# proroklab/DVM-SLAM

Measured on AMD Instinct MI355X. Metric: frames/sec ORB extract+match 640x480x8lvl, higher is better.
Workload: dtype u8; 1 GPU; single agent tracking front end: 640x480 8-level ORB extract (1000 features) + frame-to-frame windowed Hamming match, one agent per GPU; frames_per_launch_group=256, resident_stream_frames=1024, nfeatures=1000, nlevels=8, ini_th_fast=20, min_th_fast=7, match=SearchByProjection(Cur,Last) window th=15, parallelism=agents1, pipeline_lanes=2, stream_texture=rich

## Files before the change

### dvm_slam_amd/csrc/capi.cpp

```cpp
#include <algorithm>
#include <cstring>
#include <new>
#include <string>
#include <type_traits>
#include <mutex>
#include <unordered_map>
#include <vector>

#include "../../include/dvmslam_hip.h"
#include "camera_model.h"
#include "chain.h"
#include "match_kernels.h"
#include "orb_pipeline.h"

namespace dvm {
const char* last_error_cstr();
}
using namespace dvm;

struct dvm_orb {
  OrbPipeline* p;
  float* d_scale = nullptr;
  uint64_t id = 0, serial = 0;
  int last_n = 0;
// ... 84 lines not shown
  if (rc == DVM_OK) h->last_n = nn;
  return rc;
}
int dvm_orb_last_result(dvm_orb* h, dvm_device_frame* out) {
  if (!h || !out) return DVM_ERR_INVALID;
  if (!h->p->configured || h->last_n < 0 || !h->id) { set_error("dvm_orb_last_result: no single-frame result on this handle"); return DVM_ERR_STATE; }
  OrbPipeline& P = *h->p;
  out->d_kps = reinterpret_cast<const dvm_keypoint*>(P.d_kps); out->d_desc = P.d_desc;
  out->n = h->last_n; out->device = P.device; out->handle_id = h->id; out->serial = h->serial;
  return DVM_OK;
}
int dvm_device_frame_valid(const dvm_device_frame* ref) {
  if (!ref || !ref->handle_id || !ref->d_kps) return 0;
  std::lock_guard<std::mutex> l(g_orb_live_mu);
  const auto it = g_orb_live.find(ref->handle_id);
  return it != g_orb_live.end() && it->second == ref->serial ? 1 : 0;
}
int dvm_orb_extract_batch_device(dvm_orb* h, const uint8_t* d_imgs, int batch, int rows, int cols, int stride,
                                 int64_t frame_stride, int lap0, int lap1) {
  if (!h) return DVM_ERR_INVALID;
  orb_result_changed(h, -1);
  return h->p->extract_device(d_imgs, batch, rows, cols, stride, frame_stride, lap0, lap1);
}
int dvm_orb_extract_batch_host(dvm_orb* h, const uint8_t* imgs, int batch, int rows, int cols, int stride,
                               int64_t frame_stride, int lap0, int lap1) {
  if (!h) return DVM_ERR_INVALID;
  orb_result_changed(h, -1);
  return h->p->extract_host(imgs, batch, rows, cols, stride, frame_stride, lap0, lap1);
}
int dvm_orb_staging(dvm_orb* h, int batch, int rows, int cols, uint8_t** host_ptr) {
  if (!h) return DVM_ERR_INVALID;
  return h->p->staging(batch, rows, cols, host_ptr);
}
int dvm_orb_extract_staged(dvm_orb* h, int batch, int rows, int cols, int lap0, int lap1) {
  if (!h) return DVM_ERR_INVALID;
  orb_result_changed(h, -1);
  return h->p->extract_staged(batch, rows, cols, lap0, lap1);
}
int dvm_orb_sync(dvm_orb* h) { return h ? h->p->sync() : DVM_ERR_INVALID; }
int dvm_orb_result_device(dvm_orb* h, int frame, const dvm_keypoint** d_kps, const uint8_t** d_desc,
                          const int32_t** d_n, int* capacity) {
  if (!h || !h->p->configured || frame < 0 || frame >= h->p->max_batch) return DVM_ERR_STATE;
  OrbPipeline& P = *h->p;
  if (d_kps) *d_kps = reinterpret_cast<const dvm_keypoint*>(P.d_kps + (size_t)frame * P.PD.kp_cap);
  if (d_desc) *d_desc = P.d_desc + (size_t)frame * P.PD.kp_cap * 32;
  if (d_n) *d_n = P.d_n + frame;
  if (capacity) *capacity = P.PD.kp_cap;
  return DVM_OK;
}
int dvm_orb_copy_result(dvm_orb* h, int frame, dvm_keypoint* d_kps_dst, uint8_t* d_desc_dst, int32_t* d_n_dst) {
  if (!h || !h->p->configured || frame < 0 || frame >= h->p->max_batch || !d_kps_dst || !d_desc_dst || !d_n_dst) return DVM_ERR_STATE;
  OrbPipeline& P = *h->p;
  const size_t cap = (size_t)P.PD.kp_cap;
  int rc = hip_check(hipMemcpyAsync(d_kps_dst, P.d_kps + (size_t)frame * cap, cap * sizeof(dvm_keypoint), hipMemcpyDeviceToDevice, P.stream), "copy kps");
  if (rc == DVM_OK) rc = hip_check(hipMemcpyAsync(d_desc_dst, P.d_desc + (size_t)frame * cap * 32, cap * 32, hipMemcpyDeviceToDevice, P.stream), "copy desc");
  if (rc == DVM_OK) rc = hip_check(hipMemcpyAsync(d_n_dst, P.d_n + frame, 4, hipMemcpyDeviceToDevice, P.stream), "copy n");
  return rc;
}
const float* dvm_orb_scale_factors_device(dvm_orb* h) { return h ? h->d_scale : nullptr; }
int dvm_orb_download(dvm_orb* h, int frame, dvm_keypoint* kps, uint8_t* desc, int cap, int* n, int* mono_index) {
  if (!h) return DVM_ERR_INVALID;
  return h->p->download(frame, kps, desc, cap, n, mono_index);
}
int dvm_orb_download_batch(dvm_orb* h, int count, dvm_keypoint* const* kps, uint8_t* const* desc, const int* caps, int* n, int* mono_index) {
  if (!h || !caps) return DVM_ERR_INVALID;
  return h->p->download_batch(count, kps, desc, caps, n, mono_index);
}
int dvm_orb_pyramid(dvm_orb* h, int frame, int level, const uint8_t** d_ptr, int* rows, int* cols, int* stride) {
  if (!h || !h->p->configured) return DVM_ERR_STATE;
  OrbPipeline& P = *h->p;
  if (level < 0 || level >= P.PD.nlevels || frame < 0 || frame >= P.max_batch) return DVM_ERR_INVALID;
  const LevelDesc& L = P.PD.lv[level];
  if (d_ptr) *d_ptr = P.d_pyr + (size_t)frame * P.PD.pyr_frame_bytes + L.pyr_off + (size_t)kEdge * L.stride + kEdge;
  if (rows) *rows = L.h;
  if (cols) *cols = L.w;
  if (stride) *stride = L.stride;
  return DVM_OK;
}

int dvm_orb_debug_level(dvm_orb* h, int frame, int level, int bordered, uint8_t* out) {
  if (!h || !h->p->configured || !out) return DVM_ERR_STATE;
  OrbPipeline& P = *h->p;
  if (level < 0 || level >= P.PD.nlevels || frame < 0 || frame >= P.last_batch) return DVM_ERR_INVALID;
  int rc = P.sync();
  if (rc != DVM_OK) return rc;
  const LevelDesc& L = P.PD.lv[level];
  const uint8_t* base = P.d_pyr + (size_t)frame * P.PD.pyr_frame_bytes + L.pyr_off;
  if (bordered)
    return hip_check(hipMemcpy2D(out, L.w + 2 * kEdge, base, L.stride, L.w + 2 * kEdge, L.h + 2 * kEdge, hipMemcpyDeviceToHost), "memcpy2d");
  return hip_check(hipMemcpy2D(out, L.w, base + (size_t)kEdge * L.stride + kEdge, L.stride, L.w, L.h, hipMemcpyDeviceToHost), "memcpy2d");
}
int dvm_orb_debug_blurred(dvm_orb* h, int frame, int level, uint8_t* out) {
  if (!h || !h->p->configured || !out) return DVM_ERR_STATE;
  OrbPipeline& P = *h->p;
  if (level < 0 || level >= P.PD.nlevels || frame < 0 || frame >= P.last_batch) return DVM_ERR_INVALID;
  int rc = P.refresh_blur();
  if (rc == DVM_OK) rc = P.sync();
  if (rc != DVM_OK) return rc;
  const LevelDesc& L = P.PD.lv[level];
  return hip_check(hipMemcpy2D(out, L.w, P.d_blur + (size_t)frame * P.PD.blur_frame_bytes + L.blur_off, L.blur_stride, L.w, L.h,
                               hipMemcpyDeviceToHost), "memcpy2d");
}
int dvm_orb_debug_candidates(dvm_orb* h, int frame, int level, int32_t* xs, int32_t* ys, int32_t* scores, int cap, int* n) {
  if (!h || !h->p->configured) return DVM_ERR_STATE;
  OrbPipeline& P = *h->p;
  if (level < 0 || level >= P.PD.nlevels || frame < 0 || frame >= P.last_batch) return DVM_ERR_INVALID;
  int rc = P.sync();
  if (rc != DVM_OK) return rc;
  const LevelDesc& LD = P.PD.lv[level];
  std::vector<int32_t> cc(std::max(LD.cell_count, 1));
// ... 57 lines not shown
  h->p->prof.enabled = enable != 0;
  h->p->prof.only_fast = enable == 2;
  return DVM_OK;
}
int dvm_orb_profile_get(dvm_orb* h, const char* name, double* total_ms, int64_t* launches) {
  if (!h || !name) return DVM_ERR_INVALID;
  if (total_ms) *total_ms = 0;
  if (launches) *launches = 0;
  return h->p->prof.get(name, total_ms, launches) ? DVM_OK : DVM_ERR_STATE;
}
int dvm_orb_profile_reset(dvm_orb* h) {
  if (!h) return DVM_ERR_INVALID;
  h->p->prof.reset();
  return DVM_OK;
}
void* dvm_orb_stream(dvm_orb* h) { return h ? (void*)h->p->stream : nullptr; }

int dvm_hamming_matrix(const uint8_t* A, int nA, const uint8_t* B, int nB, uint16_t* D, int on_device, void* stream) {
  if (nA < 0 || nB < 0 || (nA && !A) || (nB && !B)) return DVM_ERR_INVALID;
  if (nA == 0 || nB == 0) return DVM_OK;
  if (!D) return DVM_ERR_INVALID;
  int rc = need_device(0);
  if (on_device) {
    if (rc == DVM_ERR_NO_DEVICE) return rc;
    launch_hamming_matrix((hipStream_t)stream, A, nA, B, nB, D);
    return hip_check(hipGetLastError(), "hamming launch");
  }
  if (rc != DVM_OK) return rc;
  Stage st;
  const int iA = st.in(A, (size_t)nA * 32), iB = st.in(B, (size_t)nB * 32), oD = st.out(D, (size_t)nA * nB * 2);
  rc = st.upload();
  if (rc != DVM_OK) return rc;
  launch_hamming_matrix(nullptr, st.ptr<uint8_t>(iA), nA, st.ptr<uint8_t>(iB), nB, st.ptr<uint16_t>(oD));
  rc = hip_check(hipGetLastError(), "hamming launch");
  return rc == DVM_OK ? st.download() : rc;
}

int dvm_frame_create(int device, int capacity, int slots, dvm_frame** out) {
  if (!out || capacity < 1 || capacity > kFrameCap || slots < 1) {
    set_error("dvm_frame_create: capacity must be 1..8192, slots >= 1");
    return DVM_ERR_INVALID;
  }
  *out = nullptr;
  int rc = need_device(device);
  if (rc != DVM_OK) return rc;
  dvm_frame* f = new dvm_frame{};
  f->device = device; f->cap = capacity; f->slots = slots;
  FrameView& V = f->view;
  V.cap = capacity;
  const size_t S = (size_t)slots;
  rc = hip_check(hipMalloc(&V.skp, S * capacity * sizeof(float4)), "hipMalloc");
  if (rc == DVM_OK) rc = hip_check(hipMalloc(&V.sidx, S * capacity * 4), "hipMalloc");
  if (rc == DVM_OK) rc = hip_check(hipMalloc(&V.sdesc, S * capacity * 32), "hipMalloc");
  if (rc == DVM_OK) rc = hip_check(hipMalloc(&V.cellx_start, S * 80 * 4), "hipMalloc");
  if (rc == DVM_OK) rc = hip_check(hipMalloc(&V.n_sorted, S * 4), "hipMalloc");
  if (rc == DVM_OK) rc = hip_check(hipMalloc(&V.n_total, S * 4), "hipMalloc");
  if (rc == DVM_OK) rc = hip_check(hipMalloc(&V.n_overflow, 4), "hipMalloc");
  if (rc == DVM_OK) rc = hip_check(hipMemset(V.n_overflow, 0, 4), "memset");
  if (rc == DVM_OK) rc = hip_check(hipMemset(V.cellx_start, 0, S * 80 * 4), "memset");
  if (rc == DVM_OK) rc = hip_check(hipMemset(V.n_sorted, 0, S * 4), "memset");
  if (rc == DVM_OK) rc = hip_check(hipMemset(V.n_total, 0, S * 4), "memset");
  if (rc != DVM_OK) {
    dvm_frame_destroy(f);
    return rc;
  }
  *out = f;
  return DVM_OK;
}
void dvm_frame_destroy(dvm_frame* f) {
  if (!f) return;
  FrameView& V = f->view;
  if (V.skp) hipFree(V.skp);
  if (V.sidx) hipFree(V.sidx);
  if (V.sdesc) hipFree(V.sdesc);
  if (V.cellx_start) hipFree(V.cellx_start);
  if (V.n_sorted) hipFree(V.n_sorted);
  if (V.n_total) hipFree(V.n_total);
  if (V.n_overflow) hipFree(V.n_overflow);
  if (f->d_scratch) hipFree(f->d_scratch);
  delete f;
}
static int frame_bounds(dvm_frame* f, float minX, float maxX, float minY, float maxY) {
  if (!(maxX > minX) || !(maxY > minY)) {
    set_error("frame bounds empty");
    return DVM_ERR_INVALID;
  }
  FrameView& V = f->view;
  V.minX = minX; V.minY = minY;
  V.wInv = static_cast<float>(64) / static_cast<float>(maxX - minX);
  V.hInv = static_cast<float>(48) / static_cast<float>(maxY - minY);
  return DVM_OK;
}
int dvm_frame_build(dvm_frame* f, int slot, const dvm_keypoint* kps, const uint8_t* desc, int n, const int32_t* d_n,
                    float minX, float maxX, float minY, float maxY, int on_device, void* stream) {
  if (!f || slot < 0 || slot >= f->slots || n < 0 || n > f->cap || (n && (!kps || !desc))) return DVM_ERR_INVALID;
  int rc = frame_bounds(f, minX, maxX, minY, maxY);
  if (rc != DVM_OK) return rc;
  rc = hip_check(hipSetDevice(f->device), "hipSetDevice");
  if (rc != DVM_OK) return rc;
  if (on_device) {
    launch_frame_build((hipStream_t)stream, reinterpret_cast<const dvm_keypoint_pod*>(kps), 0, desc, 0, n, d_n, f->view, slot, 1);
    return hip_check(hipGetLastError(), "frame_build launch");
  }
  Stage st;
  const int iK = st.in_mapped(kps, (size_t)n * sizeof(dvm_keypoint)), iD = st.in_mapped(desc, (size_t)n * 32);
  rc = st.upload();
  if (rc != DVM_OK) return rc;
  launch_frame_build(st.stream(), st.ptr<dvm_keypoint_pod>(iK), 0, st.ptr<uint8_t>(iD), 0, n, nullptr, f->view, slot, 1);
  rc = hip_check(hipGetLastError(), "frame_build launch");
  return rc == DVM_OK ? hip_check(hipStreamSynchronize(st.stream()), "frame_build") : rc;
}
int dvm_frame_overflows(dvm_frame* f, int32_t* count) {
  if (!f || !count) return DVM_ERR_INVALID;
  int rc = hip_check(hipSetDevice(f->device), "hipSetDevice");
  if (rc != DVM_OK) return rc;
  rc = hip_check(hipMemcpy(count, f->view.n_overflow, 4, hipMemcpyDeviceToHost), "memcpy");
  if (rc != DVM_OK) return rc;
  if (*count) { set_error("frame grid: a device-side keypoint count exceeded the handle's capacity and was truncated"); return DVM_ERR_CAPACITY; }
  return DVM_OK;
}

int dvm_frame_build_batch(dvm_frame* f, int first_slot, int count, const dvm_keypoint* d_kps, int64_t kps_stride,
                          const uint8_t* d_desc, int64_t desc_stride, const int32_t* d_n, float minX, float maxX,
                          float minY, float maxY, void* stream) {
  if (!f || first_slot < 0 || count < 1 || first_slot + count > f->slots || !d_kps || !d_desc || !d_n) return DVM_ERR_INVALID;
  int rc = frame_bounds(f, minX, maxX, minY, maxY);
  if (rc != DVM_OK) return rc;
  launch_frame_build((hipStream_t)stream, reinterpret_cast<const dvm_keypoint_pod*>(d_kps), kps_stride, d_desc, desc_stride, 0,
// ... 814 lines not shown
```

### dvm_slam_amd/csrc/fuse_targets.cpp

```cpp
#include <cstring>
#include <new>
#include <string>

#include "../../include/dvmslam_hip.h"
#include "chain.h"
#include "fuse_targets_kernels.h"
#include "orb_pipeline.h"

using namespace dvm;

struct dvm_fuse_targets : Chain {
  size_t tgt_bytes = 0, grid_bytes = 0, pts_bytes = 0, res_bytes = 0;
  int max_points = 0, max_targets = 0, max_total = 0;
  int n_targets = -1;
  int build_timed = 0;
  float last_ms[2] = {0, 0};
};

namespace {
using Cursor64 = Cursor<64>;
constexpr int kMaxTargets = 65535;
constexpr int64_t kMaxEntries = (int64_t)1 << 27;
constexpr size_t kUpPerKeypoint = sizeof(dvm_keypoint_pod) + 32, kUpFixed = 2 * 64 * 4 + 4 * 64;
constexpr size_t kGridPerKeypoint = sizeof(float4) + 4 + 32, kGridFixed = 80 * 4 + 5 * 64;
constexpr size_t kPointBytes = 12 + 12 + 4 + 4 + 32 + 1;

int fail(const char* fn, int rc, const std::string& msg) { set_error(std::string(fn) + ": " + msg); return rc; }
}

extern "C" {

int dvm_fuse_targets_create(int device, dvm_fuse_targets** out) { return chain_create(device, out); }
void dvm_fuse_targets_destroy(dvm_fuse_targets* h) { chain_destroy(h); }

int dvm_fuse_targets_reserve(dvm_fuse_targets* h, int max_points, int max_targets, int max_total_target_keypoints) {
  if (!h || max_points < 0 || max_targets < 0 || max_targets > kMaxTargets || max_total_target_keypoints < 0 ||
      (int64_t)max_total_target_keypoints > (int64_t)max_targets * kFrameCap || (int64_t)max_points * max_targets > kMaxEntries)
    return fail("dvm_fuse_targets_reserve", DVM_ERR_INVALID, "bad sizes");
  if (max_points <= h->max_points && max_targets <= h->max_targets && max_total_target_keypoints <= h->max_total) return DVM_OK;
  DVM_HIP(hipSetDevice(h->device));
  DVM_HIP(hipStreamSynchronize(h->s));
  const int np = std::max(max_points, h->max_points), nt = std::max(max_targets, h->max_targets), tot = std::max(max_total_target_keypoints, h->max_total);
  if ((int64_t)np * nt > kMaxEntries) return fail("dvm_fuse_targets_reserve", DVM_ERR_INVALID, "bad sizes");
  h->tgt_bytes = h->grid_bytes = h->pts_bytes = h->res_bytes = 0; h->max_points = h->max_targets = h->max_total = 0; h->n_targets = -1;
  const size_t tgt = pad<64>(pad<64>((size_t)nt * sizeof(FtTargetDev)) + (size_t)tot * kUpPerKeypoint + (size_t)nt * kUpFixed);
  const size_t grid = pad<64>((size_t)tot * kGridPerKeypoint + (size_t)nt * kGridFixed + 64);
  const size_t pts = pad<64>((size_t)np * kPointBytes + 7 * 64 + pad<64>((size_t)np * nt));
  const size_t res = 2 * pad<64>((size_t)np * nt * 4);
  if (const char* what = h->ws.alloc(tgt + grid + pts + res, tgt + pts + res, tgt,  false,  false))
    return fail("dvm_fuse_targets_reserve", DVM_ERR_HIP, std::string(what) + " failed");
  h->tgt_bytes = tgt; h->grid_bytes = grid; h->pts_bytes = pts; h->res_bytes = res;
  h->max_points = np; h->max_targets = nt; h->max_total = tot;
  return DVM_OK;
}

int dvm_fuse_targets_profiling(dvm_fuse_targets* h, int enable) {
  if (!h) return DVM_ERR_INVALID;
  DVM_HIP(hipSetDevice(h->device));
  return h->timer.enable(enable != 0);
}
int dvm_fuse_targets_last_kernel_ms(dvm_fuse_targets* h, float* ms) {
  if (!h || !ms) return DVM_ERR_INVALID;
  ms[0] = h->last_ms[0]; ms[1] = h->last_ms[1];
  return DVM_OK;
}

int dvm_fuse_targets_set(dvm_fuse_targets* h, int n_targets, const dvm_ft_target* targets) {
  static_assert(sizeof(dvm_keypoint) == sizeof(dvm_keypoint_pod), "layout");
  const char* fn = "dvm_fuse_targets_set";
  if (!h || n_targets < 0 || (n_targets > 0 && !targets)) return fail(fn, DVM_ERR_INVALID, "missing argument");
  int64_t total = 0;
  for (int t = 0; t < n_targets; t++) {
    const dvm_ft_target& k = targets[t];
    const std::string w = "target " + std::to_string(t);
    if (k.n < 0 || k.n > kFrameCap) return fail(fn, DVM_ERR_INVALID, w + ": n outside [0, 8192]");
    if (k.n_levels < 1 || k.n_levels > 64) return fail(fn, DVM_ERR_INVALID, w + ": n_levels outside [1, 64]");
    if (!k.scale_factors || !k.inv_level_sigma2) return fail(fn, DVM_ERR_INVALID, w + ": missing level table");
    if (!(k.fx != 0.0f) || !(k.fy != 0.0f)) return fail(fn, DVM_ERR_INVALID, w + ": zero focal length");
    if (!(k.max_x > k.min_x) || !(k.max_y > k.min_y)) return fail(fn, DVM_ERR_INVALID, w + ": image bounds empty");
    if (k.n > 0 && (!k.kps || !k.desc)) return fail(fn, DVM_ERR_INVALID, w + ": missing keypoint array");
    for (int i = 0; i < k.n; i++)
      if ((uint32_t)k.kps[i].octave >= (uint32_t)k.n_levels) return fail(fn, DVM_ERR_INVALID, w + ": a keypoint's octave outside the level tables");
    total += k.n;
  }
  if (n_targets > h->max_targets || total > h->max_total)
    return fail(fn, DVM_ERR_CAPACITY, "beyond the reservation (dvm_fuse_targets_reserve): " + std::to_string(n_targets) + " targets with " +
                                          std::to_string(total) + " keypoints");
  h->n_targets = n_targets;
  if (n_targets == 0) return DVM_OK;
  DVM_HIP(hipSetDevice(h->device));
  DVM_HIP(hipStreamSynchronize(h->s));

  const WorkingSet& ws = h->ws;
  Cursor64 up{ws.hm, ws.d};
  Cursor64 grid{ws.d + h->tgt_bytes};
  FtTargetDev* tab = up.carve<FtTargetDev>((size_t)n_targets);
  int32_t* n_overflow = grid.carve<int32_t>(1);
  for (int t = 0; t < n_targets; t++) {
    const dvm_ft_target& k = targets[t];
    FtTargetDev& D = tab[t];
    std::memset(&D, 0, sizeof(D));
    const size_t n = (size_t)k.n;
    D.kps = reinterpret_cast<const dvm_keypoint_pod*>(up.put(k.kps, n * sizeof(dvm_keypoint_pod)));
    D.desc = up.put(k.desc, n * 32);
    D.sf = reinterpret_cast<const float*>(up.put(k.scale_factors, (size_t)k.n_levels * 4));
    D.inv_sigma2 = reinterpret_cast<const float*>(up.put(k.inv_level_sigma2, (size_t)k.n_levels * 4));
    D.n = k.n;
    FrameView& F = D.F;
    F.skp = grid.carve<float4>(n);
    F.sidx = grid.carve<int32_t>(n);
    F.sdesc = grid.carve<uint8_t>(n * 32);
    F.cellx_start = grid.carve<int32_t>(80);
    F.n_sorted = grid.carve<int32_t>(2);
    F.n_total = F.n_sorted + 1;
    F.n_overflow = n_overflow;
    F.cap = k.n;
    F.minX = k.min_x; F.minY = k.min_y;
    F.wInv = static_cast<float>(64) / static_cast<float>(k.max_x - k.min_x);
    F.hInv = static_cast<float>(48) / static_cast<float>(k.max_y - k.min_y);
    ProjectCam& C = D.C;
    std::memcpy(C.q, k.Tcw.q, 16); std::memcpy(C.t, k.Tcw.t, 12); std::memcpy(C.Ow, k.Ow, 12);
    C.fx = k.fx; C.fy = k.fy; C.cx = k.cx; C.cy = k.cy;
    C.min_x = k.min_x; C.max_x = k.max_x; C.min_y = k.min_y; C.max_y = k.max_y;
    C.log_scale_factor = k.log_scale_factor; C.n_levels = k.n_levels; C.sim3_pair = 0;
  }
  if (up.used() > h->tgt_bytes || grid.used() > h->grid_bytes) return fail(fn, DVM_ERR_STATE, "packed targets exceed the reserved regions");
  DVM_HIP(hipMemcpyAsync(ws.d, ws.hm, up.used(), hipMemcpyHostToDevice, h->s));
  DVM_HIP(h->timer.mark(0, h->s));
  launch_ft_build(h->s, reinterpret_cast<const FtTargetDev*>(ws.d), n_targets);
  DVM_HIP(h->timer.mark(1, h->s));
  h->build_timed = h->timer.on;
  return hip_check(hipGetLastError(), "dvm_fuse_targets_set launch");
}

int dvm_fuse_targets_run(dvm_fuse_targets* h, const dvm_ft_points* P, const uint8_t* skip, float th, int32_t* best_idx, int32_t* best_dist) {
  const char* fn = "dvm_fuse_targets_run";
  if (!h || !P) return fail(fn, DVM_ERR_INVALID, "missing argument");
  if (h->n_targets < 0) return fail(fn, DVM_ERR_INVALID, "no targets (dvm_fuse_targets_set comes first)");
  if (P->n < 0) return fail(fn, DVM_ERR_INVALID, "negative point count");
  if (P->n > h->max_points) return fail(fn, DVM_ERR_CAPACITY, "beyond the reservation (dvm_fuse_targets_reserve): " + std::to_string(P->n) + " points");
  const int T = h->n_targets, n = P->n;
  if (T == 0 || n == 0) return DVM_OK;
  if (!P->pos || !P->normal || !P->min_dist || !P->max_dist || !P->desc || !best_idx) return fail(fn, DVM_ERR_INVALID, "missing array");
  DVM_HIP(hipSetDevice(h->device));
  const size_t N = (size_t)n, E = N * (size_t)T;
  const WorkingSet& ws = h->ws;
  uint8_t* stage = ws.hm + h->tgt_bytes;
  uint8_t* dev = ws.d + h->tgt_bytes + h->grid_bytes;
  Cursor64 up{stage, dev};
  FtPoints A{};
  A.pos = reinterpret_cast<const float*>(up.put(P->pos, N * 12));
  A.normal = reinterpret_cast<const float*>(up.put(P->normal, N * 12));
  A.min_dist = reinterpret_cast<const float*>(up.put(P->min_dist, N * 4));
  A.max_dist = reinterpret_cast<const float*>(up.put(P->max_dist, N * 4));
  A.desc = up.put(P->desc, N * 32);
  A.valid = P->valid ? up.put(P->valid, N) : nullptr;
  A.skip = skip ? up.put(skip, E) : nullptr;
  A.n = n;
  if (up.used() > h->pts_bytes) return fail(fn, DVM_ERR_STATE, "packed points exceed the reserved region");
  int32_t* d_idx = reinterpret_cast<int32_t*>(dev + h->pts_bytes);
  int32_t* d_dist = reinterpret_cast<int32_t*>(dev + h->pts_bytes + pad<64>(E * 4));
  uint8_t* h_res = stage + h->pts_bytes;
  const size_t back = best_dist ? pad<64>(E * 4) + E * 4 : E * 4;

  DVM_HIP(hipMemcpyAsync(dev, stage, up.used(), hipMemcpyHostToDevice, h->s));
// ... 20 lines not shown
```

### dvm_slam_amd/csrc/match_device.h

```cpp
#pragma once
#include <hip/hip_runtime.h>
#include <stdint.h>

#include "match_kernels.h"

namespace dvm {

__device__ __forceinline__ void desc_load(const uint8_t* __restrict__ base, int idx, uint32_t (&w)[8]) {
  const uint4* q = reinterpret_cast<const uint4*>(base + (size_t)idx * 32);
  const uint4 a = q[0], b = q[1];
  w[0] = a.x; w[1] = a.y; w[2] = a.z; w[3] = a.w; w[4] = b.x; w[5] = b.y; w[6] = b.z; w[7] = b.w;
}
__device__ __forceinline__ int desc_distance(const uint32_t (&w)[8], const uint8_t* __restrict__ base, int idx) {
  const uint4* td = reinterpret_cast<const uint4*>(base + (size_t)idx * 32);
  const uint4 a = td[0], b = td[1];
  return __popc(a.x ^ w[0]) + __popc(a.y ^ w[1]) + __popc(a.z ^ w[2]) + __popc(a.w ^ w[3]) +
         __popc(b.x ^ w[4]) + __popc(b.y ^ w[5]) + __popc(b.z ^ w[6]) + __popc(b.w ^ w[7]);
}

template <class T>
__device__ __forceinline__ void top2_insert(T& k1, T& k2, T k) {
  k2 = min(k2, max(k1, k));
  k1 = min(k1, k);
}

template <int LANES, class Visit>
__device__ __forceinline__ void window_scan(const FrameView& F, float x, float y, float r, int minLevel, int maxLevel, int lane, Visit visit) {
  const int nMinCellX = max(0, (int)floorf((x - F.minX - r) * F.wInv));
  const int nMaxCellX = min(kGridCols - 1, (int)ceilf((x - F.minX + r) * F.wInv));
  const int nMinCellY = max(0, (int)floorf((y - F.minY - r) * F.hInv));
  const int nMaxCellY = min(kGridRows - 1, (int)ceilf((y - F.minY + r) * F.hInv));
  const bool empty = nMinCellX >= kGridCols || nMaxCellX < 0 || nMinCellY >= kGridRows || nMaxCellY < 0;
  if (empty || nMinCellX > nMaxCellX) return;
  const bool checkLevels = (minLevel > 0) || (maxLevel >= 0);
  const int beg = F.cellx_start[nMinCellX], end = F.cellx_start[nMaxCellX + 1];
  for (int p = beg + lane; p < end; p += LANES) {
    const float4 kp = F.skp[p];
    const int oct = __float_as_int(kp.z);
    const int iy = __float_as_int(kp.w) % kGridRows;
    if (iy < nMinCellY || iy > nMaxCellY) continue;
    if (checkLevels) {
      if (oct < minLevel) continue;
      if (maxLevel >= 0 && oct > maxLevel) continue;
    }
    const float dx = kp.x - x, dy = kp.y - y;
    if (!(fabsf(dx) < r && fabsf(dy) < r)) continue;
    visit(p, oct, dx, dy);
  }
}

#define DVM_ROW_DPP(v, CTRL, OLD) (uint32_t)__builtin_amdgcn_update_dpp(OLD, (int)(v), CTRL, 0xF, 0xF, false)
__device__ __forceinline__ uint32_t row_min(uint32_t k) {
  k = min(k, DVM_ROW_DPP(k, 0xB1, -1));
  k = min(k, DVM_ROW_DPP(k, 0x4E, -1));
  k = min(k, DVM_ROW_DPP(k, 0x141, -1));
  k = min(k, DVM_ROW_DPP(k, 0x140, -1));
  return k;
}
template <class T>
__device__ __forceinline__ void top2_merge(T& k1, T& k2, T o1, T o2) {
  const T n1 = min(k1, o1), n2 = min(max(k1, o1), min(k2, o2));
  k1 = n1; k2 = n2;
}
__device__ __forceinline__ void row_top2(uint32_t& k1, uint32_t& k2) {
  top2_merge(k1, k2, DVM_ROW_DPP(k1, 0xB1, 0), DVM_ROW_DPP(k2, 0xB1, 0));
  top2_merge(k1, k2, DVM_ROW_DPP(k1, 0x4E, 0), DVM_ROW_DPP(k2, 0x4E, 0));
  top2_merge(k1, k2, DVM_ROW_DPP(k1, 0x141, 0), DVM_ROW_DPP(k2, 0x141, 0));
  top2_merge(k1, k2, DVM_ROW_DPP(k1, 0x140, 0), DVM_ROW_DPP(k2, 0x140, 0));
}
#undef DVM_ROW_DPP
__device__ __forceinline__ uint32_t wave_min(uint32_t k) {
#pragma unroll
  for (int o = 32; o >= 1; o >>= 1) k = min(k, (uint32_t)__shfl_xor((int)k, o));
  return k;
}
template <class T>
__device__ __forceinline__ void wave_top2(T& k1, T& k2) {
#pragma unroll
  for (int o = 32; o >= 1; o >>= 1) {
    const T o1 = __shfl_xor(k1, o), o2 = __shfl_xor(k2, o);
    top2_merge(k1, k2, o1, o2);
  }
}
__device__ __forceinline__ int wave_sum(int v) {
#pragma unroll
  for (int o = 32; o >= 1; o >>= 1) v += __shfl_xor(v, o);
  return v;
}
__device__ __forceinline__ void block_sum4_put(int v, int* s4) {
  v = wave_sum(v);
  if ((threadIdx.x & 63) == 0) s4[threadIdx.x >> 6] = v;
}
__device__ __forceinline__ int block_sum4(const int* s4) { return s4[0] + s4[1] + s4[2] + s4[3]; }

template <class ORDER>
__device__ __forceinline__ int fv_find(const int32_t* __restrict__ fv_node, int fv_n, int32_t node) {
  int lo = 0, hi = fv_n;
  while (lo < hi) {
    const int mid = (lo + hi) >> 1;
    if ((ORDER)fv_node[mid] < (ORDER)node) lo = mid + 1; else hi = mid;
// ... 33 lines not shown
```

### dvm_slam_amd/csrc/match_kernels.h

```cpp
#pragma once
#include <hip/hip_runtime.h>
#include <stdint.h>

#include "orb_kernels.h"
#include "tri_model.h"
#include "undistort_f64.h"

struct dvm_frame;

namespace dvm {

constexpr int kFrameCap = 8192;

struct dvm_match_pod {
  int32_t best_idx, best_dist, second_dist;
  int16_t best_level, second_level;
};

constexpr int kGridCols = 64, kGridRows = 48;

struct FrameView {
  float4* skp;
  int32_t* sidx;
  uint8_t* sdesc;
  int32_t* cellx_start;
  int32_t* n_sorted;
  int32_t* n_total;
  int32_t* n_overflow;
  int32_t cap;
  float minX, minY, wInv, hInv;
  __host__ __device__ FrameView slot(int s) const {
    FrameView v = *this;
    v.skp += (int64_t)s * cap;
    v.sidx += (int64_t)s * cap;
    v.sdesc += (int64_t)s * cap * 32;
    v.cellx_start += (int64_t)s * 80;
    v.n_sorted += s;
    v.n_total += s;
    return v;
  }
};

struct PairQueries {
  const dvm_keypoint_pod* kps;
  const uint8_t* desc;
  const int32_t* n;
  int64_t kps_stride, desc_stride;
  const dvm_keypoint_pod* carry_kps;
  const uint8_t* carry_desc;
  const int32_t* carry_n;
  int32_t* n_out;
  int32_t cap;
};

struct FrustumFrame {
  float Rcw[9], tcw[3], Ow[3], fx, fy, cx, cy, min_x, max_x, min_y, max_y, bf, log_scale_factor;
  int32_t n_levels;
};
struct TrackPoint {
  float proj_x, proj_y, proj_xr, depth, view_cos;
  int32_t level, in_view;
};
struct TriPair {
  double cos_parallax_max;
  float K1[4], K2[4], T1w[12], T2w[12], Ow1[3], Ow2[3];
  float ratio_factor, th_far;
  int32_t far_points, n_levels;
};
struct ProjectCam {
  float q[4], t[3];
  float Ow[3], fx, fy, cx, cy, min_x, max_x, min_y, max_y, log_scale_factor;
  int32_t n_levels;
  int32_t sim3_pair;
  float q2[4], t2[3];
  float th;
};
struct Projection {
  float u, v, radius;
  int32_t level;
};
struct CamParams {
  float p[8];
};
struct TriGeom {
  float F12[9], ep[2];
  int32_t coarse, th_low;
};
struct TriGeomKB8 {
  float ep[2];
// ... 57 lines not shown
```

### dvm_slam_amd/csrc/orb_kernels.h

```cpp
#pragma once
#include <hip/hip_runtime.h>
#include <stdint.h>

#include "orb_device.h"

namespace dvm {

struct dvm_keypoint_pod {
  float x, y, size, angle, response;
  int32_t octave, class_id;
};

struct HostMirror {
  dvm_keypoint_pod* kps = nullptr;
  uint8_t* desc = nullptr;
  int32_t* n = nullptr;
  int32_t* mono = nullptr;
};

void upload_constants(const int8_t* disc_u, const int8_t* disc_v, const int* gauss7);
void launch_pyr_level0(hipStream_t s, const uint8_t* d_src, int rows, int cols, int sstride, int64_t frame_stride,
                       uint8_t* d_pyr, const PipelineDesc& PD, int batch);
void launch_pyr_resize(hipStream_t s, uint8_t* d_pyr, const PipelineDesc& PD, int level, const int32_t* d_tabs, int batch);
void launch_pyr_borders(hipStream_t s, uint8_t* d_pyr, const PipelineDesc& PD, int batch);
void launch_fast(hipStream_t s, const uint8_t* d_pyr, const CellDesc* d_cells, const PipelineDesc& PD, uint32_t* d_cand,
                 int32_t* d_cell_count, int batch, int max_rw, int max_rh, int cell_first, int cell_num, const CellDesc* h_cells);
int octree_root_nodes(const LevelDesc& L);
bool raise_dynamic_lds(const void* fn, int bytes);
bool octree_fits_device(const PipelineDesc& PD);
bool octree_prepare_device(const PipelineDesc& PD);
void launch_octree(hipStream_t s, const uint32_t* d_cand, const int32_t* d_cell_count, const CellDesc* d_cells, uint32_t* d_dense,
                   int32_t* d_lvl_count, const PipelineDesc& PD, int32_t* d_nid, uint32_t* d_sel, int32_t* d_nsel, int32_t* d_err,
                   int batch, int level_first, int level_num, bool latency = false);
bool octree_blur_fits(const PipelineDesc& PD);
void launch_octree_blur(hipStream_t s, const uint32_t* d_cand, const int32_t* d_cell_count, const CellDesc* d_cells, uint32_t* d_dense,
                        int32_t* d_lvl_count, const PipelineDesc& PD, int32_t* d_nid, uint32_t* d_sel, int32_t* d_nsel, int32_t* d_err, int batch,
                        const uint8_t* d_pyr, uint8_t* d_blur, const TileDesc* d_tiles, const int* gauss7);
void launch_assemble(hipStream_t s, const uint32_t* d_sel, const int32_t* d_nsel, const PipelineDesc& PD, int lap0,
                     int lap1, dvm_keypoint_pod* d_kps, KpAux* d_aux, int32_t* d_n, int32_t* d_mono, int batch,
                     HostMirror hm = HostMirror());
void launch_blur(hipStream_t s, const uint8_t* d_pyr, uint8_t* d_blur, const TileDesc* d_tiles, const PipelineDesc& PD,
                 const int32_t* d_lvl_start, int batch);
void launch_orient_desc(hipStream_t s, const uint8_t* d_pyr, const uint8_t* d_blur, const PipelineDesc& PD,
                        const KpAux* d_aux, const int32_t* d_n, dvm_keypoint_pod* d_kps, uint8_t* d_desc, int batch,
                        HostMirror hm = HostMirror());
void launch_orient_desc_blur(hipStream_t s, const uint8_t* d_pyr, const PipelineDesc& PD, const KpAux* d_aux, const int32_t* d_n,
                             dvm_keypoint_pod* d_kps, uint8_t* d_desc, int batch, HostMirror hm = HostMirror());

}
```

### dvm_slam_amd/csrc/orb_kernels.hip

```cpp
#include <hip/hip_runtime.h>

#include <map>
#include <mutex>
#include <utility>

#include <algorithm>
#include <cstdlib>

#include "orb_device.h"
#include "orb_kernels.h"
#include "blur_tile.h"

#pragma clang fp contract(off)

namespace dvm {

__constant__ int c_pattern[1024] = {
#include "orb_pattern_31.inc"
};
__constant__ int8_t c_circle[16][2] = {{0, 3},  {1, 3},   {2, 2},   {3, 1},   {3, 0},  {3, -1}, {2, -2}, {1, -3},
                                       {0, -3}, {-1, -3}, {-2, -2}, {-3, -1}, {-3, 0}, {-3, 1}, {-2, 2}, {-1, 3}};
__device__ uint2 c_disc_w[256];
__device__ uint2 c_disc_w43[512];
__constant__ int c_gauss7[7];
// ... 1321 lines not shown
  if (!h_cells || lds1_max <= 0) { launch_fast_wide(s, d_pyr, d_cells, PD, d_cand, d_cell_count, batch, max_rw, max_rh, cell_first, cell_num); return; }
  const int end = cell_first + cell_num;
  int run_first = cell_first, run_kind = -1, run_rw = 0, run_rh = 0;
  auto flush = [&](int upto) {
    if (upto <= run_first || run_kind < 0) return;
    const int n = upto - run_first;
    if (run_kind == 0) { launch_fast_wide(s, d_pyr, d_cells, PD, d_cand, d_cell_count, batch, run_rw, run_rh, run_first, n); return; }
    const int pitch = run_kind;
    const int lds = fast1_lds_layout(pitch, run_rw, run_rh).total();
    const dim3 grid(n * 8 * ((batch + 8 * kFastFramesPerWG - 1) / (8 * kFastFramesPerWG)));
    if (pitch == 48)
      hipLaunchKernelGGL((k_fast_cells1<48>), grid, dim3(64), lds, s, d_pyr, PD.pyr_frame_bytes, d_cells, PD, d_cand, d_cell_count, run_rw, run_rh, batch, run_first, n);
    else
      hipLaunchKernelGGL((k_fast_cells1<64>), grid, dim3(64), lds, s, d_pyr, PD.pyr_frame_bytes, d_cells, PD, d_cand, d_cell_count, run_rw, run_rh, batch, run_first, n);
  };
  int c = cell_first;
  while (c < end) {
    const int lvl = h_cells[c].level;
    int e = c, rw = 8, rh = 8;
    for (; e < end && h_cells[e].level == lvl; e++) { rw = std::max<int>(rw, h_cells[e].rw); rh = std::max<int>(rh, h_cells[e].rh); }
    const int pitch = fast1_pick_pitch(rw);
    const int kind = pitch != 0 && fast1_lds_layout(pitch, rw, rh).total() <= (pitch == 48 ? lds1_max : lds1_max64) ? pitch : 0;
    if (kind != 0 && kind == run_kind) {
      const int jrw = std::max(run_rw, rw), jrh = std::max(run_rh, rh);
      if (fast1_lds_layout(kind, jrw, jrh).total() > (kind == 48 ? lds1_max : lds1_max64)) { flush(c); run_first = c; run_kind = -1; }
    }
    if (kind != run_kind) { flush(c); run_first = c; run_kind = kind; run_rw = rw; run_rh = rh; }
    else { run_rw = std::max(run_rw, rw); run_rh = std::max(run_rh, rh); }
    c = e;
  }
  flush(end);
}
void launch_assemble(hipStream_t s, const uint32_t* d_sel, const int32_t* d_nsel, const PipelineDesc& PD, int lap0,
                     int lap1, dvm_keypoint_pod* d_kps, KpAux* d_aux, int32_t* d_n, int32_t* d_mono, int batch, HostMirror hm) {
  hipLaunchKernelGGL(k_assemble, dim3(batch), dim3(256), 0, s, d_sel, d_nsel, PD, lap0, lap1, d_kps, d_aux, d_n, d_mono, hm);
}
void launch_blur(hipStream_t s, const uint8_t* d_pyr, uint8_t* d_blur, const TileDesc* d_tiles, const PipelineDesc& PD,
                 const int32_t* d_lvl_start, int batch) {
  hipLaunchKernelGGL(k_blur7, dim3(xcd_grid(PD.ntiles, batch)), dim3(256), 0, s, d_pyr, PD.pyr_frame_bytes, d_blur,
                     PD.blur_frame_bytes, d_tiles, PD, d_lvl_start, batch);
}
void launch_orient_desc(hipStream_t s, const uint8_t* d_pyr, const uint8_t* d_blur, const PipelineDesc& PD,
                        const KpAux* d_aux, const int32_t* d_n, dvm_keypoint_pod* d_kps, uint8_t* d_desc, int batch, HostMirror hm) {
  hipLaunchKernelGGL(k_orient_desc, dim3(xcd_grid(cdiv(PD.kp_cap, 4 * kDescPerWave), batch)), dim3(256), 0, s, d_pyr, PD.pyr_frame_bytes,
                     d_blur, PD.blur_frame_bytes, PD, d_aux, d_n, d_kps, d_desc, batch, hm);
}

void launch_orient_desc_blur(hipStream_t s, const uint8_t* d_pyr, const PipelineDesc& PD, const KpAux* d_aux, const int32_t* d_n,
                             dvm_keypoint_pod* d_kps, uint8_t* d_desc, int batch, HostMirror hm) {
  hipLaunchKernelGGL(k_orient_desc_blur, dim3(xcd_grid(cdiv(PD.kp_cap, 4 * kPbPerWave), batch)), dim3(256), 0, s, d_pyr, PD.pyr_frame_bytes, PD,
                     d_aux, d_n, d_kps, d_desc, batch, hm);
}

}
```

### dvm_slam_amd/csrc/proj_device.h

```cpp
#pragma once
#include <hip/hip_runtime.h>
#include <stdint.h>

#include "camera_model.h"
#include "match_device.h"
#include "match_kernels.h"
#include "pose_f32.h"

namespace dvm {

constexpr uint32_t kInvalidKey = 0xFFFFFFFFu;

__device__ __forceinline__ void frame_build_block(const dvm_keypoint_pod* __restrict__ kps, const uint8_t* __restrict__ desc, int n,
                                                  const FrameView& F) {
  __shared__ uint32_t keys[kFrameCap];
  const int tid = threadIdx.x;
  int P = 64;
  while (P < n) P <<= 1;
  for (int i = tid; i < P; i += 1024) {
    uint32_t key = kInvalidKey;
    if (i < n) {
      const dvm_keypoint_pod kp = kps[i];
      int px = (int)roundf((kp.x - F.minX) * F.wInv);
      int py = (int)roundf((kp.y - F.minY) * F.hInv);
      if (px >= 0 && px < kGridCols && py >= 0 && py < kGridRows) key = ((uint32_t)(px * kGridRows + py) << 13) | (uint32_t)i;
    }
    keys[i] = key;
  }
  __syncthreads();
  for (int k = 2; k <= P; k <<= 1) {
    for (int j = k >> 1; j > 0; j >>= 1) {
      for (int i = tid; i < P; i += 1024) {
        int ixj = i ^ j;
        if (ixj > i) {
          uint32_t a = keys[i], b = keys[ixj];
          bool up = ((i & k) == 0);
          if ((a > b) == up) { keys[i] = b; keys[ixj] = a; }
        }
      }
      const int jn = j > 1 ? (j >> 1) : k;
      if (j >= 64 || jn >= 64) {
        __syncthreads();
      } else {
        __builtin_amdgcn_fence(__ATOMIC_ACQ_REL, "wavefront");
        __builtin_amdgcn_wave_barrier();
      }
    }
  }
  __shared__ int s_m;
  if (tid == 0) {
    int lo = 0, hi = P;
    while (lo < hi) {
      int mid = (lo + hi) >> 1;
      if (keys[mid] == kInvalidKey) hi = mid; else lo = mid + 1;
    }
    s_m = lo;
    *F.n_sorted = lo;
    *F.n_total = n;
  }
  __syncthreads();
  const int m = s_m;
  if (tid <= kGridCols) {
    uint32_t want = (uint32_t)(tid * kGridRows) << 13;
    int lo = 0, hi = m;
    while (lo < hi) {
      int mid = (lo + hi) >> 1;
      if (keys[mid] < want) lo = mid + 1; else hi = mid;
    }
    F.cellx_start[tid] = lo;
  }
  for (int p = tid; p < m; p += 1024) {
    const uint32_t key = keys[p];
    const int i = (int)(key & 0x1FFFu);
    const dvm_keypoint_pod kp = kps[i];
    F.skp[p] = make_float4(kp.x, kp.y, __int_as_float(kp.octave), __int_as_float((int)(key >> 13)));
    F.sidx[p] = i;
    const uint4* s = reinterpret_cast<const uint4*>(desc + (size_t)i * 32);
    uint4* d = reinterpret_cast<uint4*>(F.sdesc + (size_t)p * 32);
    d[0] = s[0];
    d[1] = s[1];
  }
}

__device__ __forceinline__ void window_top2(const FrameView& F, float x, float y, float r, int minLevel, int maxLevel,
                                            const uint8_t* __restrict__ qdesc32, const uint8_t* __restrict__ skip,
                                            const float* __restrict__ gate_inv_sigma2, double gate, int lane, uint32_t& k1_out,
                                            uint32_t& k2_out) {
  uint32_t k1 = (256u << 16) | 0xFFFFu, k2 = k1;
  uint32_t w[8];
  desc_load(qdesc32, 0, w);
  window_scan<16>(F, x, y, r, minLevel, maxLevel, lane, [&](int p, int oct, float dx, float dy) {
    if (skip && skip[F.sidx[p]]) return;
    if (gate_inv_sigma2) {
      const float e2 = __fadd_rn(__fmul_rn(dx, dx), __fmul_rn(dy, dy));
      if ((double)__fmul_rn(e2, gate_inv_sigma2[oct]) > gate) return;
    }
    top2_insert(k1, k2, ((uint32_t)desc_distance(w, F.sdesc, p) << 16) | (uint32_t)p);
  });
  row_top2(k1, k2);
  k1_out = k1; k2_out = k2;
}

struct ProjectRow {
  uint32_t k1, k2;
  float u, v, r;
  int level;
};
template <int MODEL = dvm_cam::kPinhole>
__device__ __forceinline__ ProjectRow project_row(const FrameView& F, const uint8_t* __restrict__ skip, const ProjectCam& C, float th,
                                                  const float* __restrict__ P, const float* __restrict__ normal,
                                                  const float* __restrict__ min_dist, const float* __restrict__ max_dist,
                                                  const uint8_t* __restrict__ desc, bool ok, int i, const float* __restrict__ scale_factors,
                                                  const float* __restrict__ gate_inv_sigma2, double gate, int lane,
                                                  const float* kb8 = nullptr) {
  float out_u = -1.f, out_v = -1.f, out_r = 0.f;
  int out_level = -1;
  const float p0 = P[3 * i], p1 = P[3 * i + 1], p2 = P[3 * i + 2];
  const float pw[3] = {p0, p1, p2};
  float pc[3];
  dvm_pose::se3_apply(C.q, C.t, pw, pc);
  float X = pc[0], Y = pc[1], Z = pc[2];
  float u, v;
// ... 48 lines not shown
```

Measured before the change: 291,100 frames/s.

## Index match grid per cell and compact window candidates via DPP prefix queue

Replaces the per-column start index with a full per-cell start table built with a branchless binary search, so window scans visit only keypoints in the covered rows of each column. A wave-level DPP prefix sum compacts candidate indices into a shared-memory queue so lanes work on dense candidate lists rather than filtering whole columns. Also replaces the three device-to-device memcpys in result copying with a single vectorized copy kernel. It adds shared memory use, wave barriers and a larger cell table in exchange for fewer wasted keypoint loads.

```diff
diff --git a/dvm_slam_amd/csrc/capi.cpp b/dvm_slam_amd/csrc/capi.cpp
--- a/dvm_slam_amd/csrc/capi.cpp
+++ b/dvm_slam_amd/csrc/capi.cpp
@@ -160,10 +160,11 @@
   if (!h || !h->p->configured || frame < 0 || frame >= h->p->max_batch || !d_kps_dst || !d_desc_dst || !d_n_dst) return DVM_ERR_STATE;
   OrbPipeline& P = *h->p;
   const size_t cap = (size_t)P.PD.kp_cap;
-  int rc = hip_check(hipMemcpyAsync(d_kps_dst, P.d_kps + (size_t)frame * cap, cap * sizeof(dvm_keypoint), hipMemcpyDeviceToDevice, P.stream), "copy kps");
-  if (rc == DVM_OK) rc = hip_check(hipMemcpyAsync(d_desc_dst, P.d_desc + (size_t)frame * cap * 32, cap * 32, hipMemcpyDeviceToDevice, P.stream), "copy desc");
-  if (rc == DVM_OK) rc = hip_check(hipMemcpyAsync(d_n_dst, P.d_n + frame, 4, hipMemcpyDeviceToDevice, P.stream), "copy n");
-  return rc;
+  int rc = hip_check(hipSetDevice(P.device), "hipSetDevice");
+  if (rc != DVM_OK) return rc;
+  launch_copy_result(P.stream, P.d_kps + (size_t)frame * cap, reinterpret_cast<dvm_keypoint_pod*>(d_kps_dst), P.d_desc + (size_t)frame * cap * 32, d_desc_dst,
+                     (int)cap, P.d_n + frame, d_n_dst);
+  return hip_check(hipGetLastError(), "copy_result launch");
 }
 const float* dvm_orb_scale_factors_device(dvm_orb* h) { return h ? h->d_scale : nullptr; }
 int dvm_orb_download(dvm_orb* h, int frame, dvm_keypoint* kps, uint8_t* desc, int cap, int* n, int* mono_index) {
@@ -327,12 +328,12 @@
   rc = hip_check(hipMalloc(&V.skp, S * capacity * sizeof(float4)), "hipMalloc");
   if (rc == DVM_OK) rc = hip_check(hipMalloc(&V.sidx, S * capacity * 4), "hipMalloc");
   if (rc == DVM_OK) rc = hip_check(hipMalloc(&V.sdesc, S * capacity * 32), "hipMalloc");
-  if (rc == DVM_OK) rc = hip_check(hipMalloc(&V.cellx_start, S * 80 * 4), "hipMalloc");
+  if (rc == DVM_OK) rc = hip_check(hipMalloc(&V.cell_start, S * kCellStartStride * 4), "hipMalloc");
   if (rc == DVM_OK) rc = hip_check(hipMalloc(&V.n_sorted, S * 4), "hipMalloc");
   if (rc == DVM_OK) rc = hip_check(hipMalloc(&V.n_total, S * 4), "hipMalloc");
   if (rc == DVM_OK) rc = hip_check(hipMalloc(&V.n_overflow, 4), "hipMalloc");
   if (rc == DVM_OK) rc = hip_check(hipMemset(V.n_overflow, 0, 4), "memset");
-  if (rc == DVM_OK) rc = hip_check(hipMemset(V.cellx_start, 0, S * 80 * 4), "memset");
+  if (rc == DVM_OK) rc = hip_check(hipMemset(V.cell_start, 0, S * kCellStartStride * 4), "memset");
   if (rc == DVM_OK) rc = hip_check(hipMemset(V.n_sorted, 0, S * 4), "memset");
   if (rc == DVM_OK) rc = hip_check(hipMemset(V.n_total, 0, S * 4), "memset");
   if (rc != DVM_OK) {
@@ -348,7 +349,7 @@
   if (V.skp) hipFree(V.skp);
   if (V.sidx) hipFree(V.sidx);
   if (V.sdesc) hipFree(V.sdesc);
-  if (V.cellx_start) hipFree(V.cellx_start);
+  if (V.cell_start) hipFree(V.cell_start);
   if (V.n_sorted) hipFree(V.n_sorted);
   if (V.n_total) hipFree(V.n_total);
   if (V.n_overflow) hipFree(V.n_overflow);
diff --git a/dvm_slam_amd/csrc/fuse_targets.cpp b/dvm_slam_amd/csrc/fuse_targets.cpp
--- a/dvm_slam_amd/csrc/fuse_targets.cpp
+++ b/dvm_slam_amd/csrc/fuse_targets.cpp
@@ -22,7 +22,7 @@
 constexpr int kMaxTargets = 65535;
 constexpr int64_t kMaxEntries = (int64_t)1 << 27;
 constexpr size_t kUpPerKeypoint = sizeof(dvm_keypoint_pod) + 32, kUpFixed = 2 * 64 * 4 + 4 * 64;
-constexpr size_t kGridPerKeypoint = sizeof(float4) + 4 + 32, kGridFixed = 80 * 4 + 5 * 64;
+constexpr size_t kGridPerKeypoint = sizeof(float4) + 4 + 32, kGridFixed = (size_t)kCellStartStride * 4 + 5 * 64;
 constexpr size_t kPointBytes = 12 + 12 + 4 + 4 + 32 + 1;
 
 int fail(const char* fn, int rc, const std::string& msg) { set_error(std::string(fn) + ": " + msg); return rc; }
@@ -110,7 +110,7 @@
     F.skp = grid.carve<float4>(n);
     F.sidx = grid.carve<int32_t>(n);
     F.sdesc = grid.carve<uint8_t>(n * 32);
-    F.cellx_start = grid.carve<int32_t>(80);
+    F.cell_start = grid.carve<int32_t>(kCellStartStride);
     F.n_sorted = grid.carve<int32_t>(2);
     F.n_total = F.n_sorted + 1;
     F.n_overflow = n_overflow;
diff --git a/dvm_slam_amd/csrc/match_device.h b/dvm_slam_amd/csrc/match_device.h
--- a/dvm_slam_amd/csrc/match_device.h
+++ b/dvm_slam_amd/csrc/match_device.h
@@ -24,6 +24,28 @@
   k1 = min(k1, k);
 }
 
+#define DVM_ROW_SHR(v, N) __builtin_amdgcn_update_dpp(0, v, 0x110 + N, 0xF, 0xF, false)
+template <int LANES>
+__device__ __forceinline__ int lanes_prefix(int v, int lane) {
+  static_assert(LANES == 16 || LANES == 64, "a DPP row or the wave");
+  v += DVM_ROW_SHR(v, 1);
+  v += DVM_ROW_SHR(v, 2);
+  v += DVM_ROW_SHR(v, 4);
+  v += DVM_ROW_SHR(v, 8);
+  if constexpr (LANES == 64) {
+    const int t0 = __builtin_amdgcn_readlane(v, 15), t1 = __builtin_amdgcn_readlane(v, 31), t2 = __builtin_amdgcn_readlane(v, 47);
+    v += (lane >= 16 ? t0 : 0) + (lane >= 32 ? t1 : 0) + (lane >= 48 ? t2 : 0);
+  }
+  return v;
+}
+#undef DVM_ROW_SHR
+template <int LANES>
+__device__ __forceinline__ int lanes_total(int incl) {
+  if constexpr (LANES == 64) return __builtin_amdgcn_readlane(incl, 63);
+  else return __builtin_amdgcn_update_dpp(0, incl, 0x15F, 0xF, 0xF, false);
+}
+
+constexpr int kWindowQueue = 4;
 template <int LANES, class Visit>
 __device__ __forceinline__ void window_scan(const FrameView& F, float x, float y, float r, int minLevel, int maxLevel, int lane, Visit visit) {
   const int nMinCellX = max(0, (int)floorf((x - F.minX - r) * F.wInv));
@@ -31,21 +53,42 @@
   const int nMinCellY = max(0, (int)floorf((y - F.minY - r) * F.hInv));
   const int nMaxCellY = min(kGridRows - 1, (int)ceilf((y - F.minY + r) * F.hInv));
   const bool empty = nMinCellX >= kGridCols || nMaxCellX < 0 || nMinCellY >= kGridRows || nMaxCellY < 0;
-  if (empty || nMinCellX > nMaxCellX) return;
+  if (empty || nMinCellX > nMaxCellX || nMinCellY > nMaxCellY) return;
   const bool checkLevels = (minLevel > 0) || (maxLevel >= 0);
-  const int beg = F.cellx_start[nMinCellX], end = F.cellx_start[nMaxCellX + 1];
-  for (int p = beg + lane; p < end; p += LANES) {
-    const float4 kp = F.skp[p];
-    const int oct = __float_as_int(kp.z);
-    const int iy = __float_as_int(kp.w) % kGridRows;
-    if (iy < nMinCellY || iy > nMaxCellY) continue;
-    if (checkLevels) {
-      if (oct < minLevel) continue;
-      if (maxLevel >= 0 && oct > maxLevel) continue;
+  constexpr int kQueue = kWindowQueue * LANES;
+  __shared__ uint16_t s_queue[(256 / LANES) * kQueue];
+  uint16_t* queue = s_queue + (threadIdx.x / LANES) * kQueue;
+  for (int g = nMinCellX; g <= nMaxCellX; g += LANES) {
+    const int c = g + lane;
+    int beg = 0, len = 0;
+    if (c <= nMaxCellX) {
+      beg = F.cell_start[c * kGridRows + nMinCellY];
+      len = F.cell_start[c * kGridRows + nMaxCellY + 1] - beg;
     }
-    const float dx = kp.x - x, dy = kp.y - y;
-    if (!(fabsf(dx) < r && fabsf(dy) < r)) continue;
-    visit(p, oct, dx, dy);
+    const int incl = lanes_prefix<LANES>(len, lane), excl = incl - len;
+    const int total = lanes_total<LANES>(incl);
+    for (int base = 0; base < total; base += kQueue) {
+      const int hi = min(incl, base + kQueue);
+#pragma clang loop vectorize(disable) unroll(disable)
+      for (int f = max(excl, base); f < hi; f++) queue[f - base] = (uint16_t)(beg + (f - excl));
+      __builtin_amdgcn_fence(__ATOMIC_ACQ_REL, "wavefront");
+      __builtin_amdgcn_wave_barrier();
+      const int n = min(total - base, kQueue);
+      for (int j = lane; j < n; j += LANES) {
+        const int p = queue[j];
+        const float4 kp = F.skp[p];
+        const int oct = __float_as_int(kp.z);
+        if (checkLevels) {
+          if (oct < minLevel) continue;
+          if (maxLevel >= 0 && oct > maxLevel) continue;
+        }
+        const float dx = kp.x - x, dy = kp.y - y;
+        if (!(fabsf(dx) < r && fabsf(dy) < r)) continue;
+        visit(p, oct, dx, dy);
+      }
+      __builtin_amdgcn_fence(__ATOMIC_ACQ_REL, "wavefront");
+      __builtin_amdgcn_wave_barrier();
+    }
   }
 }
 
diff --git a/dvm_slam_amd/csrc/match_kernels.h b/dvm_slam_amd/csrc/match_kernels.h
--- a/dvm_slam_amd/csrc/match_kernels.h
+++ b/dvm_slam_amd/csrc/match_kernels.h
@@ -18,12 +18,14 @@
 };
 
 constexpr int kGridCols = 64, kGridRows = 48;
+constexpr int kGridCells = kGridCols * kGridRows;
+constexpr int kCellStartStride = kGridCells + 4;
 
 struct FrameView {
   float4* skp;
   int32_t* sidx;
   uint8_t* sdesc;
-  int32_t* cellx_start;
+  int32_t* cell_start;
   int32_t* n_sorted;
   int32_t* n_total;
   int32_t* n_overflow;
@@ -34,7 +36,7 @@
     v.skp += (int64_t)s * cap;
     v.sidx += (int64_t)s * cap;
     v.sdesc += (int64_t)s * cap * 32;
-    v.cellx_start += (int64_t)s * 80;
+    v.cell_start += (int64_t)s * kCellStartStride;
     v.n_sorted += s;
     v.n_total += s;
     return v;
diff --git a/dvm_slam_amd/csrc/orb_kernels.h b/dvm_slam_amd/csrc/orb_kernels.h
--- a/dvm_slam_amd/csrc/orb_kernels.h
+++ b/dvm_slam_amd/csrc/orb_kernels.h
@@ -46,5 +46,7 @@
                         HostMirror hm = HostMirror());
 void launch_orient_desc_blur(hipStream_t s, const uint8_t* d_pyr, const PipelineDesc& PD, const KpAux* d_aux, const int32_t* d_n,
                              dvm_keypoint_pod* d_kps, uint8_t* d_desc, int batch, HostMirror hm = HostMirror());
+void launch_copy_result(hipStream_t s, const dvm_keypoint_pod* kps_src, dvm_keypoint_pod* kps_dst, const uint8_t* desc_src, uint8_t* desc_dst, int cap,
+                        const int32_t* n_src, int32_t* n_dst);
 
 }
diff --git a/dvm_slam_amd/csrc/orb_kernels.hip b/dvm_slam_amd/csrc/orb_kernels.hip
--- a/dvm_slam_amd/csrc/orb_kernels.hip
+++ b/dvm_slam_amd/csrc/orb_kernels.hip
@@ -1397,4 +1397,29 @@
                      d_aux, d_n, d_kps, d_desc, batch, hm);
 }
 
-}
+template <class W>
+__global__ void __launch_bounds__(256) k_copy_result(const W* __restrict__ kps_src, W* __restrict__ kps_dst, uint32_t n_kps,
+                                                     const W* __restrict__ desc_src, W* __restrict__ desc_dst, uint32_t n_desc,
+                                                     const int32_t* __restrict__ n_src, int32_t* __restrict__ n_dst) {
+  const uint32_t i = blockIdx.x * 256 + threadIdx.x;
+  if (i < n_kps) kps_dst[i] = kps_src[i];
+  else if (i - n_kps < n_desc) desc_dst[i - n_kps] = desc_src[i - n_kps];
+  if (i == 0) *n_dst = *n_src;
+}
+template <class W>
+static void copy_result_as(hipStream_t s, const void* kps_src, void* kps_dst, size_t kps_bytes, const void* desc_src, void* desc_dst,
+                           size_t desc_bytes, const int32_t* n_src, int32_t* n_dst) {
+  const uint32_t nk = (uint32_t)(kps_bytes / sizeof(W)), nd = (uint32_t)(desc_bytes / sizeof(W));
+  hipLaunchKernelGGL(k_copy_result<W>, dim3(max(1, cdiv((int)(nk + nd), 256))), dim3(256), 0, s, static_cast<const W*>(kps_src), static_cast<W*>(kps_dst), nk,
+                     static_cast<const W*>(desc_src), static_cast<W*>(desc_dst), nd, n_src, n_dst);
+}
+void launch_copy_result(hipStream_t s, const dvm_keypoint_pod* kps_src, dvm_keypoint_pod* kps_dst, const uint8_t* desc_src, uint8_t* desc_dst, int cap,
+                        const int32_t* n_src, int32_t* n_dst) {
+  const size_t kb = (size_t)cap * sizeof(dvm_keypoint_pod), db = (size_t)cap * 32;
+  const uintptr_t a = (uintptr_t)kps_src | (uintptr_t)kps_dst | (uintptr_t)desc_src | (uintptr_t)desc_dst | kb | db;
+  if (a % 16 == 0) copy_result_as<uint4>(s, kps_src, kps_dst, kb, desc_src, desc_dst, db, n_src, n_dst);
+  else if (a % 4 == 0) copy_result_as<uint32_t>(s, kps_src, kps_dst, kb, desc_src, desc_dst, db, n_src, n_dst);
+  else copy_result_as<uint8_t>(s, kps_src, kps_dst, kb, desc_src, desc_dst, db, n_src, n_dst);
+}
+
+}
diff --git a/dvm_slam_amd/csrc/proj_device.h b/dvm_slam_amd/csrc/proj_device.h
--- a/dvm_slam_amd/csrc/proj_device.h
+++ b/dvm_slam_amd/csrc/proj_device.h
@@ -60,14 +60,20 @@
   }
   __syncthreads();
   const int m = s_m;
-  if (tid <= kGridCols) {
-    uint32_t want = (uint32_t)(tid * kGridRows) << 13;
-    int lo = 0, hi = m;
-    while (lo < hi) {
-      int mid = (lo + hi) >> 1;
-      if (keys[mid] < want) lo = mid + 1; else hi = mid;
+  {
+    const uint32_t w0 = (uint32_t)tid << 13, w1 = (uint32_t)(tid + 1024) << 13, w2 = (uint32_t)(tid + 2048) << 13;
+    int l0 = 0, l1 = 0, l2 = 0;
+    for (int s = P; s > 0; s >>= 1) {
+      const bool in0 = l0 + s <= P, in1 = l1 + s <= P, in2 = l2 + s <= P;
+      const uint32_t k0 = keys[in0 ? l0 + s - 1 : 0], k1 = keys[in1 ? l1 + s - 1 : 0], k2 = keys[in2 ? l2 + s - 1 : 0];
+      if (in0 && k0 < w0) l0 += s;
+      if (in1 && k1 < w1) l1 += s;
+      if (in2 && k2 < w2) l2 += s;
     }
-    F.cellx_start[tid] = lo;
+    F.cell_start[tid] = l0;
+    F.cell_start[tid + 1024] = l1;
+    F.cell_start[tid + 2048] = l2;
+    if (tid == 0) F.cell_start[kGridCells] = m;
   }
   for (int p = tid; p < m; p += 1024) {
     const uint32_t key = keys[p];
```

After: 300,700 frames/s, median of 6. +3.3%, better.
